# wenet-e2e/wekws

Hardware: AMD Instinct MI355X
Metric: 1-sec utterances/sec (40-d fbank -> DS-TCN posteriors), whole job; per-frame streaming latency in `latency` (higher is better)
Workload: dtype f32 in/out/accumulate; products as 3 x fp16 MFMA on block-floating hi/lo-split operands (fp32-level accuracy at any operand scale); 1 GPU; ds_tcn_h256 forward, 1024 x 1-s utterances per GPU, T=98 frames x 40-d fbank in HBM -> (B,98,2) posteriors + the streaming cache; batch_per_gpu=1024, frames=98, feat_dim=40, precision=f16x3, preheat_steps=2450, parallelism=utterance-parallel x1

## Files before the change

wekws_amd/csrc/ds256_g16.hip.h:

```cpp
#pragma once
#include <utility>

#include "ds256_w16.hip.h"

namespace wekws {

#ifdef WEKWS_G16_STAMPS
#define G16_PH_DECL long long tph[8] = {0, 0, 0, 0, 0, 0, 0, 0}; long long tlast = clock64()
#define G16_PH(id) do { long long now_ = clock64(); tph[id] += now_ - tlast; tlast = now_; } while (0)
#define G16_PH_DUMP                                                                                    \
  do {                                                                                                 \
    __syncthreads();                                                                                   \
    if (blockIdx.x == 0 && A.out_cache && (threadIdx.x & 63) == 0)                                    \
      for (int i = 0; i < 8; ++i) A.out_cache[(threadIdx.x >> 6) * 8 + i] = float(tph[i]);               \
  } while (0)
#else
#define G16_PH_DECL
#define G16_PH(id)
#define G16_PH_DUMP
#endif

template <int S>
__device__ __forceinline__ void g16_fmac_shr(float& o, float x, float w) {
  static_assert(S >= 1 && S <= 15, "row shift");
#define G16_SHR(n) if constexpr (S == n) asm("v_fmac_f32_dpp %0, %1, %2 row_shr:" #n " row_mask:0xf bank_mask:0xf" : "+v"(o) : "v"(x), "v"(w));
  G16_SHR(1) G16_SHR(2) G16_SHR(3) G16_SHR(4) G16_SHR(5) G16_SHR(6) G16_SHR(7) G16_SHR(8)
  G16_SHR(9) G16_SHR(10) G16_SHR(11) G16_SHR(12) G16_SHR(13) G16_SHR(14) G16_SHR(15)
#undef G16_SHR
}
template <int S, int TT_, int NT, int R_>
__device__ __forceinline__ void g16_tap(float& o, const f32x4 (&hv)[NT], float w) {
  constexpr int Q = S / NT, M = S % NT;
  constexpr int REG = TT_ >= M ? TT_ - M : TT_ - M + NT;
  constexpr int SH = TT_ >= M ? Q : Q + 1;
  if constexpr (SH == 0) o = fmaf(w, hv[REG][R_], o);
  else if constexpr (SH <= 15) g16_fmac_shr<SH>(o, hv[REG][R_], w);
}
template <int S, int NT, int R_, int... TTs>
__device__ __forceinline__ void g16_tap_tiles(float (&o)[NT], const f32x4 (&hv)[NT], float w, std::integer_sequence<int, TTs...>) {
  (g16_tap<S, TTs, NT, R_>(o[TTs], hv, w), ...);
}

template <int S>
__device__ __forceinline__ void g16_fmac_shl(float& o, float x, float w) {
  static_assert(S >= 1 && S <= 15, "row shift");
#define G16_SHL(n) if constexpr (S == n) asm("v_fmac_f32_dpp %0, %1, %2 row_shl:" #n " row_mask:0xf bank_mask:0xf" : "+v"(o) : "v"(x), "v"(w));
  G16_SHL(1) G16_SHL(2) G16_SHL(3) G16_SHL(4) G16_SHL(5) G16_SHL(6) G16_SHL(7) G16_SHL(8)
  G16_SHL(9) G16_SHL(10) G16_SHL(11) G16_SHL(12) G16_SHL(13) G16_SHL(14) G16_SHL(15)
#undef G16_SHL
}
template <int S, int TT_, int NT, int R_, int PART>
__device__ __forceinline__ void g16_tapc(float& o, const f32x4 (&hv)[NT], const f32x4 (&cx)[NT], float w) {
  constexpr int Q = S / NT, M = S % NT;
  constexpr int REG = TT_ >= M ? TT_ - M : TT_ - M + NT;
  constexpr int SH = TT_ >= M ? Q : Q + 1;
  static_assert(SH <= 15, "the context is one 16-lane row: NT >= 4 for paddings up to 56 frames");
  if constexpr (SH == 0) {
    if constexpr (PART == 0) o = fmaf(w, hv[REG][R_], o);
  } else if constexpr (PART == 0) {
    g16_fmac_shr<SH>(o, hv[REG][R_], w);
  } else {
    g16_fmac_shl<16 - SH>(o, cx[REG][R_], w);
  }
}
template <int S, int NT, int R_, int... TTs>
__device__ __forceinline__ void g16_tapc_tiles(float (&o)[NT], const f32x4 (&hv)[NT], const f32x4 (&cx)[NT], float w,
                                               std::integer_sequence<int, TTs...>) {
  (g16_tapc<S, TTs, NT, R_, 0>(o[TTs], hv, cx, w), ...);
  (g16_tapc<S, TTs, NT, R_, 1>(o[TTs], hv, cx, w), ...);
}

typedef float g16_f32x2 __attribute__((ext_vector_type(2)));
typedef _Float16 g16_f16x2 __attribute__((ext_vector_type(2)));

template <bool SPLIT>
__device__ __forceinline__ void g16_split_pair(float v0, float v1, float s, unsigned& ph, unsigned& pl) {
  const float t0 = fmaxf(v0, 0.f) * s, t1 = fmaxf(v1, 0.f) * s;
  const g16_f16x2 h = __builtin_convertvector(g16_f32x2{t0, t1}, g16_f16x2);
  ph = __builtin_bit_cast(unsigned, h);
  if constexpr (SPLIT) {
    const float d0 = t0 - static_cast<float>(h[0]), d1 = t1 - static_cast<float>(h[1]);
    pl = __builtin_bit_cast(unsigned, __builtin_convertvector(g16_f32x2{d0, d1}, g16_f16x2));
  }
}

template <int D, int P_, int NT, bool SPLIT, bool CTX = false>
__device__ __forceinline__ void g16_dw_pair(const f32x4 (&hv)[NT], const f32x4 (&cx)[NT], const float* taps_o0, float sa, char* pst, int lo_off) {
  const float4* src = reinterpret_cast<const float4*>(taps_o0 + 2 * P_ * 12);
  const float4 a0 = src[0], a1 = src[1], a2 = src[2], b0 = src[3], b1 = src[4], b2 = src[5];
  constexpr auto tiles = std::make_integer_sequence<int, NT>{};
  constexpr int RA = 2 * P_, RB = 2 * P_ + 1;
  float oa[NT], ob[NT];
  __builtin_amdgcn_s_setprio(P_ == 0 ? 3 : 1);
#pragma unroll
  for (int tt = 0; tt < NT; ++tt) { oa[tt] = a2.x; ob[tt] = b2.x; }
  if constexpr (CTX) {
    g16_tapc_tiles<7 * D, NT, RA>(oa, hv, cx, a0.x, tiles); g16_tapc_tiles<7 * D, NT, RB>(ob, hv, cx, b0.x, tiles);
    g16_tapc_tiles<6 * D, NT, RA>(oa, hv, cx, a0.y, tiles); g16_tapc_tiles<6 * D, NT, RB>(ob, hv, cx, b0.y, tiles);
    g16_tapc_tiles<5 * D, NT, RA>(oa, hv, cx, a0.z, tiles); g16_tapc_tiles<5 * D, NT, RB>(ob, hv, cx, b0.z, tiles);
    g16_tapc_tiles<4 * D, NT, RA>(oa, hv, cx, a0.w, tiles); g16_tapc_tiles<4 * D, NT, RB>(ob, hv, cx, b0.w, tiles);
    g16_tapc_tiles<3 * D, NT, RA>(oa, hv, cx, a1.x, tiles); g16_tapc_tiles<3 * D, NT, RB>(ob, hv, cx, b1.x, tiles);
    g16_tapc_tiles<2 * D, NT, RA>(oa, hv, cx, a1.y, tiles); g16_tapc_tiles<2 * D, NT, RB>(ob, hv, cx, b1.y, tiles);
    g16_tapc_tiles<1 * D, NT, RA>(oa, hv, cx, a1.z, tiles); g16_tapc_tiles<1 * D, NT, RB>(ob, hv, cx, b1.z, tiles);
    g16_tapc_tiles<0, NT, RA>(oa, hv, cx, a1.w, tiles);     g16_tapc_tiles<0, NT, RB>(ob, hv, cx, b1.w, tiles);
  } else {
  g16_tap_tiles<7 * D, NT, RA>(oa, hv, a0.x, tiles); g16_tap_tiles<7 * D, NT, RB>(ob, hv, b0.x, tiles);
  g16_tap_tiles<6 * D, NT, RA>(oa, hv, a0.y, tiles); g16_tap_tiles<6 * D, NT, RB>(ob, hv, b0.y, tiles);
  g16_tap_tiles<5 * D, NT, RA>(oa, hv, a0.z, tiles); g16_tap_tiles<5 * D, NT, RB>(ob, hv, b0.z, tiles);
  g16_tap_tiles<4 * D, NT, RA>(oa, hv, a0.w, tiles); g16_tap_tiles<4 * D, NT, RB>(ob, hv, b0.w, tiles);
  g16_tap_tiles<3 * D, NT, RA>(oa, hv, a1.x, tiles); g16_tap_tiles<3 * D, NT, RB>(ob, hv, b1.x, tiles);
  g16_tap_tiles<2 * D, NT, RA>(oa, hv, a1.y, tiles); g16_tap_tiles<2 * D, NT, RB>(ob, hv, b1.y, tiles);
  g16_tap_tiles<1 * D, NT, RA>(oa, hv, a1.z, tiles); g16_tap_tiles<1 * D, NT, RB>(ob, hv, b1.z, tiles);
  g16_tap_tiles<0, NT, RA>(oa, hv, a1.w, tiles);     g16_tap_tiles<0, NT, RB>(ob, hv, b1.w, tiles);
  }
  __builtin_amdgcn_s_setprio(P_ == 0 ? 2 : 0);
#pragma unroll
  for (int tt = 0; tt < NT; ++tt) {
    unsigned ph, pl;
    g16_split_pair<SPLIT>(oa[tt], ob[tt], sa, ph, pl);
    *reinterpret_cast<unsigned*>(pst + tt * 256 + P_ * 4) = ph;
    if constexpr (SPLIT) *reinterpret_cast<unsigned*>(pst + lo_off + tt * 256 + P_ * 4) = pl;
  }
}
template <int D, int NT, bool SPLIT, bool CTX = false>
__device__ __forceinline__ void g16_dw_rows(const f32x4 (&hv)[NT], const f32x4 (&cx)[NT], const float* taps_o0, float sa, char* pst, int lo_off) {
  g16_dw_pair<D, 0, NT, SPLIT, CTX>(hv, cx, taps_o0, sa, pst, lo_off);
  g16_dw_pair<D, 1, NT, SPLIT, CTX>(hv, cx, taps_o0, sa, pst, lo_off);
}
template <int D, int NT, bool SPLIT>
__device__ __forceinline__ void g16_dw_rows(const f32x4 (&hv)[NT], const float* taps_o0, float sa, char* pst, int lo_off) {
  g16_dw_rows<D, NT, SPLIT, false>(hv, hv, taps_o0, sa, pst, lo_off);
}

template <int NT>
__device__ __forceinline__ void g16_load_run(const float* src, f32x4 (&cv)[NT], int r) {
  struct __attribute__((packed, aligned(4))) V4 { float v[4]; };
  struct __attribute__((packed, aligned(4))) V3 { float v[3]; };
  if constexpr (NT == 7) {
    const V4 a = *reinterpret_cast<const V4*>(src);
    const V3 c = *reinterpret_cast<const V3*>(src + 4);
    cv[0][r] = a.v[0]; cv[1][r] = a.v[1]; cv[2][r] = a.v[2]; cv[3][r] = a.v[3];
    cv[4][r] = c.v[0]; cv[5][r] = c.v[1]; cv[6][r] = c.v[2];
  } else if constexpr (NT == 4) {
    const V4 a = *reinterpret_cast<const V4*>(src);
    cv[0][r] = a.v[0]; cv[1][r] = a.v[1]; cv[2][r] = a.v[2]; cv[3][r] = a.v[3];
  } else {
#pragma unroll
    for (int tt = 0; tt < NT; ++tt) cv[tt][r] = src[tt];
  }
}

template <int NT, int PB>
__device__ __forceinline__ W16XItem g16_take_x(const float* xbuf, int T, int idim, int nk, int e) {
  constexpr int TT = 16 * NT;
  W16XItem it;
  const int n = e % TT, q = e / TT;
  const int f = NT * (n & 15) + (n >> 4);
  const int oct = q & 3, st = q >> 2;
  const int kf = st * 32 + oct * 8;
  const bool has = e < nk * 4 * TT;
  it.dst = has ? st * 2 * PB + (oct * TT + n) * 16 : -1;
  it.ok = has && f < T && kf < idim;
  const float* p = xbuf + (it.ok ? f * idim + kf : 0);
  const float4 a = *reinterpret_cast<const float4*>(p), c = *reinterpret_cast<const float4*>(p + 4);
  it.v = w16_f32x8{a.x, a.y, a.z, a.w, c.x, c.y, c.z, c.w};
  return it;
}

template <int NT>
__device__ __forceinline__ void g16_store_run(float* dst, const f32x4 (&hv)[NT], int r) {
  struct __attribute__((packed, aligned(4))) V4 { float v[4]; };
  struct __attribute__((packed, aligned(4))) V3 { float v[3]; };
  struct __attribute__((packed, aligned(4))) V2 { float v[2]; };
  if constexpr (NT == 7) {
    *reinterpret_cast<V4*>(dst) = V4{{hv[0][r], hv[1][r], hv[2][r], hv[3][r]}};
    *reinterpret_cast<V3*>(dst + 4) = V3{{hv[4][r], hv[5][r], hv[6][r]}};
  } else if constexpr (NT == 4) {
    *reinterpret_cast<V4*>(dst) = V4{{hv[0][r], hv[1][r], hv[2][r], hv[3][r]}};
  } else if constexpr (NT == 2) {
    *reinterpret_cast<V2*>(dst) = V2{{hv[0][r], hv[1][r]}};
  } else {
#pragma unroll
    for (int tt = 0; tt < NT; ++tt) dst[tt] = hv[tt][r];
  }
}

template <int NT, int PB>
__device__ __forceinline__ W16XItem g16_load_x(const float* __restrict__ xb, int T, int idim, int nk, int e) {
  constexpr int TT = 16 * NT;
  W16XItem it;
  const int n = e % TT, q = e / TT;
  const int f = NT * (n & 15) + (n >> 4);
  const int oct = q & 3, st = q >> 2;
  const int kf = st * 32 + oct * 8;
  const bool has = e < nk * 4 * TT;
  it.dst = has ? st * 2 * PB + (oct * TT + n) * 16 : -1;
  w16_fetch_x(it, xb + int64_t(f) * idim + kf, xb, has && f < T && kf < idim);
  return it;
}

template <int NT, bool SPLIT, bool FIRST = false>
__device__ __forceinline__ void g16_mfma_step(f32x4 (&acc)[NT], const F16Frag& a, const char* bh, const char* bl) {
  f16x8 vh[2], vl[2];
  vh[0] = *reinterpret_cast<const f16x8*>(bh);
  if constexpr (SPLIT) vl[0] = *reinterpret_cast<const f16x8*>(bl);
#pragma unroll
  for (int tt = 0; tt < NT; ++tt) {
    if (tt + 1 < NT) {
      vh[(tt + 1) & 1] = *reinterpret_cast<const f16x8*>(bh + (tt + 1) * 256);
      if constexpr (SPLIT) vl[(tt + 1) & 1] = *reinterpret_cast<const f16x8*>(bl + (tt + 1) * 256);
    }
    __builtin_amdgcn_sched_barrier(0);
    acc[tt] = __builtin_amdgcn_mfma_f32_16x16x32_f16(a.h, vh[tt & 1], FIRST ? f32x4{0.f, 0.f, 0.f, 0.f} : acc[tt], 0, 0, 0);
    if constexpr (SPLIT) {
      acc[tt] = __builtin_amdgcn_mfma_f32_16x16x32_f16(a.h, vl[tt & 1], acc[tt], 0, 0, 0);
      acc[tt] = __builtin_amdgcn_mfma_f32_16x16x32_f16(a.l, vh[tt & 1], acc[tt], 0, 0, 0);
    }
    __builtin_amdgcn_sched_barrier(0);
  }
}

template <int NT, bool SPLIT, bool FAST, bool CTX = false>
__global__ __launch_bounds__(kW16Threads) void ds256_g16_kernel(const StackParams P, const CallArgs A) {
  static_assert(!CTX || (FAST && NT >= 4), "the context tile is one 16-lane row");
  using G = W16Geom<NT>;
  constexpr int C = G::C, SS = G::SS, TT = G::TT, PB = G::PB;
  constexpr int NKS = C / 32;
  constexpr int OTS = NKS * 128;
  static_assert(size_t(2 * NKS) * PB <= G::LDS_BYTES, "the operand planes of a whole layer live where the f32 tile was");
  extern __shared__ __attribute__((aligned(16))) float w16_lds[];
  char* const planes = reinterpret_cast<char*>(w16_lds);
  float* const hbuf = w16_lds + G::SLAB / 4;

  f32x4 acc[NT];
  f32x4 hv[NT];
  f32x4 cx[CTX ? NT : 1];
  G16_PH_DECL;

  __shared__ AmaxCell amax_cells[kAmaxCells];
  __shared__ BlockDesc blk[kAmaxMaxBlocks];
  __shared__ NfList nfl;
  nf_list_init(nfl);
  __shared__ __attribute__((aligned(16))) float taps[C * 12];
  const int nk = P.kpre16 / 32;
  const bool one_trip = FAST || (nk <= 2 && 8 * TT <= kW16Threads && w16_x_vec_ok(A.x, A.xs_b, P.idim));
  static_assert(kAmaxMaxBlocks * sizeof(BlockDesc) / 4 <= kW16Threads, "one table dword per thread");
  {
    const int ntbl = P.nblocks * int(sizeof(BlockDesc) / 4);
    const int t0 = threadIdx.x;
    if (t0 < ntbl) reinterpret_cast<uint32_t*>(blk)[t0] = reinterpret_cast<const uint32_t*>(P.blocks)[t0];
  }
  float* const xbuf = w16_lds + (2 * NKS * PB) / 4;
  static_assert(!FAST || size_t(2 * NKS) * PB + size_t(TT) * 64 * 4 <= G::LDS_BYTES, "feature buffer above the planes");
  auto prefetch_x = [&](int bn) __attribute__((always_inline)) {
    const int nitems = (A.T * P.idim) >> 2;
    const float* src = A.x + int64_t(bn) * A.xs_b;
    const int t0 = threadIdx.x;
    for (int e0 = 0; e0 < nitems; e0 += kW16Threads) {
      const int wbase = __builtin_amdgcn_readfirstlane(e0 + (t0 & ~63));
      if (e0 + t0 < nitems)
        __builtin_amdgcn_global_load_lds((const __attribute__((address_space(1))) void*)(src + (e0 + t0) * 4),
                                         (__attribute__((address_space(3))) void*)(xbuf + wbase * 4), 16, 0, 0);
    }
  };
  if constexpr (FAST) prefetch_x(blockIdx.x);
  for (int b = blockIdx.x; b < A.B; b += gridDim.x) {
  const float* Wp = P.w;
  if constexpr (FAST) asm volatile("" : "+s"(Wp));
  const float* __restrict__ W = Wp;
  int tid = threadIdx.x;
  if constexpr (FAST) asm volatile("" : "+v"(tid));
  const int lane = tid & 63, wave = __builtin_amdgcn_readfirstlane(tid >> 6);
  const int l15 = lane & 15, lq = lane >> 4;
  int T = A.T;
  if constexpr (FAST) asm volatile("" : "+s"(T));
  const int Pc = P.cache_len;
  const int o0 = wave * 16 + lq * 4;
  const int frag_off = (lq * TT + l15) * 16;
  char* const pst = planes + (wave >> 1) * 2 * PB + ((((wave & 1) * 2 + (lq >> 1)) * TT + l15) * 16 + (lq & 1) * 8);

  auto stage_taps = [&](const BlockDesc& nb) __attribute__((always_inline)) {
    if (wave < C * 3 / 64)
      __builtin_amdgcn_global_load_lds((const __attribute__((address_space(1))) void*)(W + nb.dw_pk + tid * 4),
                                       (__attribute__((address_space(3))) void*)(taps + wave * 256), 16, 0, 0);
  };
  auto load_ctx = [&](int bi) __attribute__((always_inline)) {
    if constexpr (CTX) {
      const int padn = __builtin_amdgcn_readfirstlane(blk[bi].pad), offn = __builtin_amdgcn_readfirstlane(blk[bi].cache_off);
      const float* const ic = A.in_cache + (int64_t(b) * C + o0) * Pc + offn;
      const int c0 = padn + NT * (l15 - 16);
#pragma unroll
      for (int tt = 0; tt < NT; ++tt) cx[tt] = f32x4{0.f, 0.f, 0.f, 0.f};
      if (c0 >= 0) {
#pragma unroll
        for (int r = 0; r < 4; ++r) g16_load_run<NT>(ic + r * Pc + c0, cx, r);
      } else if (c0 + NT > 0) {
#pragma unroll
        for (int tt = 0; tt < NT; ++tt)
          if (c0 + tt >= 0) {
#pragma unroll
            for (int r = 0; r < 4; ++r) cx[tt][r] = ic[r * Pc + c0 + tt];
          }
      }
    }
  };
  auto skip_bad = [&]() __attribute__((always_inline)) {
    nf_list_note(nfl, b);
    if constexpr (FAST) {
      if (b + int(gridDim.x) < A.B) prefetch_x(b + gridDim.x);
    }
  };
  amax_zero<kW16Threads>(amax_cells, kAmaxCells);
  W16XItem xi;
  if constexpr (!FAST) {
    if (one_trip) xi = g16_load_x<NT, PB>(A.x + int64_t(b) * A.xs_b, T, P.idim, nk, tid);
  } else {
    __builtin_amdgcn_s_waitcnt(0x0F70);
  }
  __syncthreads();
  stage_taps(blk[0]);
  if constexpr (CTX)
    amax_publish(amax_cells + 1, amax_span_bits<kW16Threads>(A.in_cache + int64_t(b) * C * Pc, C * Pc, 0.f));
  if constexpr (FAST) xi = g16_take_x<NT, PB>(xbuf, T, P.idim, nk, tid);
  if (one_trip) {
    amax_publish(amax_cells, w16_x_amax_bits(xi));
  } else {
    amax_publish(amax_cells, amax_span_bits<kW16Threads>(A.x + int64_t(b) * A.xs_b, T * P.idim, 0.f));
  }

  {
#pragma unroll
    for (int tt = 0; tt < NT; ++tt) acc[tt] = f32x4{0.f, 0.f, 0.f, 0.f};
    const uint4* ap = reinterpret_cast<const uint4*>(W + P.pre_a16) + size_t(wave) * nk * 128 + lane;
    const float4 bias = *reinterpret_cast<const float4*>(W + P.pre_b + o0);
    float sx = 1.f, cpre = 1.f;
    if (one_trip) {
      F16Frag a[2];
#pragma unroll
      for (int st = 0; st < 2; ++st) {
        const uint4* q = ap + min(st, nk - 1) * 128;
        a[st].h = __builtin_bit_cast(f16x8, q[0]);
        a[st].l = __builtin_bit_cast(f16x8, q[64]);
      }
      __syncthreads();
      if (amax_inputs_bad(amax_cells)) { skip_bad(); continue; }
      sx = pow2_scale(amax_read(amax_cells), &cpre);
      w16_store_x<PB, SPLIT>(xi, sx, planes);
      __syncthreads();
#pragma unroll
      for (int st = 0; st < 2; ++st)
        if (st < nk)
          g16_mfma_step<NT, SPLIT>(acc, a[st], planes + st * 2 * PB + frag_off, planes + st * 2 * PB + PB + frag_off);
    } else {
    __syncthreads();
    if (amax_inputs_bad(amax_cells)) { skip_bad(); continue; }
    for (int k0 = 0; k0 < nk; k0 += 2) {
      const int steps = min(2, nk - k0);
      __syncthreads();
      sx = pow2_scale(amax_read(amax_cells), &cpre);
      for (int e = tid; e < steps * 4 * TT; e += kW16Threads) {
        const int n = e % TT;
        const int t = NT * (n & 15) + (n >> 4);
        const int q = e / TT;
        const int oct = q & 3, st = q >> 2;
        const int kf = (k0 + st) * 32 + oct * 8;
        const bool ok = t < T;
        const float* xr = A.x + int64_t(b) * A.xs_b + int64_t(t) * P.idim + kf;
        f16x8 vh, vl;
#pragma unroll
        for (int i = 0; i < 8; ++i) {
          const float v = (ok && kf + i < P.idim) ? xr[i] * sx : 0.f;
          _Float16 h, l;
          split16(v, h, l);
          vh[i] = h; vl[i] = l;
        }
        char* dst = planes + st * 2 * PB + (oct * TT + n) * 16;
        *reinterpret_cast<f16x8*>(dst) = vh;
        if constexpr (SPLIT) *reinterpret_cast<f16x8*>(dst + PB) = vl;
      }
      __syncthreads();
      for (int st = 0; st < steps; ++st) {
        F16Frag a[1];
        load_a16<1>(a, ap + (k0 + st) * 128, 0);
        g16_mfma_step<NT, SPLIT>(acc, a[0], planes + st * 2 * PB + frag_off, planes + st * 2 * PB + PB + frag_off);
      }
    }
    }
    cpre *= P.pre_inv_s;
    float hmax = 0.f;
#pragma unroll
    for (int tt = 0; tt < NT; ++tt) {
#pragma unroll
      for (int r = 0; r < 4; ++r) {
        float v = fmaf(acc[tt][r], cpre, f4c(bias, r));
        if (P.pre_relu) v = fmaxf(v, 0.f);
        hv[tt][r] = v;
        hmax = fmaxf(hmax, fabsf(v));
      }
    }
    amax_publish(amax_cells + 2, hmax);
    __syncthreads();
  }
  G16_PH(0);
  F16Frag a0;
  auto frag_base = [&](int i) __attribute__((always_inline)) {
    return reinterpret_cast<const uint4*>(W + __builtin_amdgcn_readfirstlane(blk[i].a1_16)) + size_t(wave) * OTS;
  };
  {
    const uint4* ap0 = frag_base(0);
    F16Frag t[1];
    load_a16<1>(t, ap0 + lane, 0); a0 = t[0];
  }
  for (int bi = 0; bi < P.nblocks; ++bi) {
    const BlockDesc bd = blk[bi];
    const int pad = bd.pad;
    const uint4* ap1 = frag_base(bi);
    const uint4* apn = frag_base(min(bi + 1, P.nblocks - 1));
    float c1;
    const float au = CTX ? fmaxf(amax_read(amax_cells + 2 + bi), amax_read(amax_cells + 1)) : amax_read(amax_cells + 2 + bi);
    const float sa = pow2_scale(fmaf(bd.dw_alpha, au, bd.dw_beta), &c1);
    c1 *= bd.inv_s1;

    auto hand_over = [&]() __attribute__((always_inline)) {
      if (A.out_cache) {
        float* const oc = A.out_cache + (int64_t(b) * C + o0) * Pc + bd.cache_off;
        const int p0 = NT * l15 - (T - pad);
        if (p0 >= 0 && p0 + NT <= pad) {
#pragma unroll
          for (int r = 0; r < 4; ++r) g16_store_run<NT>(oc + r * Pc + p0, hv, r);
        } else if (p0 + NT > 0 && p0 < pad) {
#pragma unroll
          for (int tt = 0; tt < NT; ++tt) {
            const int p = p0 + tt;
            if (p >= 0 && p < pad) {
#pragma unroll
              for (int r = 0; r < 4; ++r) oc[r * Pc + p] = hv[tt][r];
            }
          }
        }
        if (T < pad) {
          const int nz = pad - T;
          for (int e = lane; e < 16 * nz; e += 64) {
            const int cc = e / nz, p = e - cc * nz;
            const int64_t at = (int64_t(b) * C + wave * 16 + cc) * Pc + bd.cache_off + p;
            A.out_cache[at] = CTX ? A.in_cache[at + T] : 0.f;
          }
        }
      }
    };
    load_ctx(bi);
    G16_PH(1);

    {
      const float* taps_o0 = taps + o0 * 12;
      switch (bd.dil) {
        case 1: if constexpr (CTX) g16_dw_rows<1, NT, SPLIT, true>(hv, cx, taps_o0, sa, pst, PB); else g16_dw_rows<1, NT, SPLIT>(hv, taps_o0, sa, pst, PB); break;
        case 2: if constexpr (CTX) g16_dw_rows<2, NT, SPLIT, true>(hv, cx, taps_o0, sa, pst, PB); else g16_dw_rows<2, NT, SPLIT>(hv, taps_o0, sa, pst, PB); break;
        case 4: if constexpr (CTX) g16_dw_rows<4, NT, SPLIT, true>(hv, cx, taps_o0, sa, pst, PB); else g16_dw_rows<4, NT, SPLIT>(hv, taps_o0, sa, pst, PB); break;
        case 8: if constexpr (CTX) g16_dw_rows<8, NT, SPLIT, true>(hv, cx, taps_o0, sa, pst, PB); else g16_dw_rows<8, NT, SPLIT>(hv, taps_o0, sa, pst, PB); break;
        default: break;
      }
    }
    G16_PH(2);
    __syncthreads();
    G16_PH(3);

    F16Frag a1;
    {
      F16Frag t[1];
      load_a16<1>(t, ap1 + 128 + lane, 0); a1 = t[0];
    }
    const float4 ebias = *reinterpret_cast<const float4*>(W + bd.b1 + o0);
    if (bi + 1 < P.nblocks) stage_taps(blk[bi + 1]);

    auto kpass = [&](int ks, auto first_c) __attribute__((always_inline)) {
      if (ks == 0) __builtin_amdgcn_s_setprio(3);
      else if (ks == 2) __builtin_amdgcn_s_setprio(2);
      else if (ks == 4) __builtin_amdgcn_s_setprio(1);
      else __builtin_amdgcn_s_setprio(0);
      const char* bsrc = planes + ks * 2 * PB + frag_off;
      const uint4* nx = ks + 2 < NKS ? ap1 + (ks + 2) * 128 : apn;
      g16_mfma_step<NT, SPLIT, decltype(first_c)::value>(acc, a0, bsrc, bsrc + PB);
      {
        F16Frag t[1];
        load_a16<1>(t, nx + lane, 0); a0 = t[0];
      }
      g16_mfma_step<NT, SPLIT>(acc, a1, bsrc + 2 * PB, bsrc + 3 * PB);
      if (ks + 2 < NKS) {
        F16Frag t[1];
        load_a16<1>(t, nx + 128 + lane, 0); a1 = t[0];
      }
    };
    kpass(0, std::true_type{});
#pragma unroll 1
    for (int ks = 2; ks < NKS; ks += 2) kpass(ks, std::false_type{});
    G16_PH(4);

    hand_over();
    G16_PH(6);

    float hmax = 0.f;
#pragma unroll
    for (int tt = 0; tt < NT; ++tt) {
#pragma unroll
      for (int r = 0; r < 4; ++r) {
        const float v = fmaxf(fmaf(acc[tt][r], c1, f4c(ebias, r)), 0.f) + hv[tt][r];
        hv[tt][r] = v;
        hmax = fmaxf(hmax, fabsf(v));
      }
    }
    amax_publish(amax_cells + 3 + bi, hmax);
    G16_PH(5);
    __syncthreads();
    G16_PH(3);
  }

  if (FAST || (P.head == HEAD_LINEAR && P.odim <= 2)) {
    const int K = P.odim;
    constexpr int PS = 32 * NT + 16;
    float* const part = w16_lds;
    {
      const float4 w0 = *reinterpret_cast<const float4*>(W + P.head_w + o0);
      const float4 w1 = *reinterpret_cast<const float4*>(W + P.head_w + (K > 1 ? C : 0) + o0);
      if constexpr (FAST) {
        if (b + int(gridDim.x) < A.B) prefetch_x(b + gridDim.x);
      }
      float* dst = part + (wave * 4 + lq) * PS + 2 * NT * l15;
      const HeadPairs hw(w0, w1);
#pragma unroll
      for (int tt = 0; tt < NT; ++tt) {
        pk_f32x2 pp{0.f, 0.f};
        head_fma4(pp, hw.x, hw.y, hw.z, hw.w, hv[tt]);
        *reinterpret_cast<float2*>(dst + 2 * tt) = float2{pp.x, pp.y};
      }
    }
    __syncthreads();
    {
      const int e = tid >> 2, qd = tid & 3;
      const int t = e >> 1, k = e & 1;
      const float* src = part + qd * 16 * PS + e;
      float v = 0.f;
#pragma unroll
      for (int i = 0; i < 16; ++i) v += src[i * PS];
      v += __builtin_bit_cast(float, __builtin_amdgcn_update_dpp(0, __builtin_bit_cast(int, v), 0xB1, 0xf, 0xf, true));
      v += __builtin_bit_cast(float, __builtin_amdgcn_update_dpp(0, __builtin_bit_cast(int, v), 0x4E, 0xf, 0xf, true));
      if (qd == 0 && t < T && k < K) {
        v += W[P.head_b + k];
        if (P.sigmoid) v = sigmoidf_(v);
        A.y[int64_t(b) * A.ys_b + int64_t(t) * K + k] = v;
      }
    }
  } else if constexpr (!FAST) {
#pragma unroll
    for (int tt = 0; tt < NT; ++tt) {
#pragma unroll
      for (int r = 0; r < 4; ++r) hbuf[(o0 + r) * SS + NT * l15 + tt] = hv[tt][r];
    }
    __syncthreads();
    conv_stack_head<KIND_DS, 256, NT, kW16Threads, SS>(P, A, hbuf, w16_lds, b);
  }
  G16_PH(7);
  if constexpr (!FAST) break;
  }
  nf_list_drain(nfl, A, P.idim, C * P.cache_len, blockIdx.x, gridDim.x);
  G16_PH_DUMP;
}

int launch_ds256_g16(const Route& r, const StackParams& P, const CallArgs& A, hipStream_t stream);

}
```

Measured before the change: 5.037 million utts/s.

## Use SGPR-base plus VGPR-offset global addressing and move next-utterance prefetch earlier

Weight and feature loads now go through explicit global address-space pointers, with a uniform scalar base and a 32-bit per-lane offset. This lets the compiler emit saddr+voffset global loads instead of building 64-bit per-lane addresses. The k-loop peels its final pass so the last pass never issues the unused a1 fragment load. The tap staging for the next block is moved after the MFMA loop, and the FAST-path prefetch of the next utterance is moved from the head into the last block so it overlaps more work. The risk is that the earlier prefetch writes xbuf while it may still be read, and the moved staging changes the overlap timing.

```diff
diff --git a/wekws_amd/csrc/ds256_g16.hip.h b/wekws_amd/csrc/ds256_g16.hip.h
--- a/wekws_amd/csrc/ds256_g16.hip.h
+++ b/wekws_amd/csrc/ds256_g16.hip.h
@@ -199,6 +199,33 @@
   return it;
 }
 
+#if defined(__HIP_DEVICE_COMPILE__)
+typedef const __attribute__((address_space(1))) char* g16_gptr;
+#else
+typedef const char* g16_gptr;
+#endif
+__device__ __forceinline__ g16_gptr g16_global(const void* p) { return (g16_gptr)p; }
+template <class V>
+__device__ __forceinline__ V g16_ld(g16_gptr base, uint32_t off) {
+  asm volatile("" : "+v"(off));
+#if defined(__HIP_DEVICE_COMPILE__)
+  return *reinterpret_cast<const __attribute__((address_space(1))) V*>(base + off);
+#else
+  return *reinterpret_cast<const V*>(base + off);
+#endif
+}
+__device__ __forceinline__ g16_gptr g16_sect(g16_gptr w, uint32_t at) { return w + int64_t(at) * 4; }
+__device__ __forceinline__ uint32_t g16_voff(uint32_t off) {
+  asm volatile("" : "+v"(off));
+  return off;
+}
+__device__ __forceinline__ F16Frag g16_frag(g16_gptr base, uint32_t lane_off) {
+  F16Frag a;
+  a.h = g16_ld<f16x8>(base, lane_off);
+  a.l = g16_ld<f16x8>(base + 64 * 16, lane_off);
+  return a;
+}
+
 template <int NT, bool SPLIT, bool FIRST = false>
 __device__ __forceinline__ void g16_mfma_step(f32x4 (&acc)[NT], const F16Frag& a, const char* bh, const char* bl) {
   f16x8 vh[2], vl[2];
@@ -254,20 +281,20 @@
   static_assert(!FAST || size_t(2 * NKS) * PB + size_t(TT) * 64 * 4 <= G::LDS_BYTES, "feature buffer above the planes");
   auto prefetch_x = [&](int bn) __attribute__((always_inline)) {
     const int nitems = (A.T * P.idim) >> 2;
-    const float* src = A.x + int64_t(bn) * A.xs_b;
+    const g16_gptr src = g16_global(A.x + int64_t(bn) * A.xs_b);
     const int t0 = threadIdx.x;
     for (int e0 = 0; e0 < nitems; e0 += kW16Threads) {
       const int wbase = __builtin_amdgcn_readfirstlane(e0 + (t0 & ~63));
       if (e0 + t0 < nitems)
-        __builtin_amdgcn_global_load_lds((const __attribute__((address_space(1))) void*)(src + (e0 + t0) * 4),
+        __builtin_amdgcn_global_load_lds(src + int64_t(wbase) * 16 + g16_voff(uint32_t(t0 & 63) * 16),
                                          (__attribute__((address_space(3))) void*)(xbuf + wbase * 4), 16, 0, 0);
     }
   };
   if constexpr (FAST) prefetch_x(blockIdx.x);
   for (int b = blockIdx.x; b < A.B; b += gridDim.x) {
-  const float* Wp = P.w;
-  if constexpr (FAST) asm volatile("" : "+s"(Wp));
-  const float* __restrict__ W = Wp;
+  g16_gptr Wg = g16_global(P.w);
+  if constexpr (FAST) asm volatile("" : "+s"(Wg));
+
   int tid = threadIdx.x;
   if constexpr (FAST) asm volatile("" : "+v"(tid));
   const int lane = tid & 63, wave = __builtin_amdgcn_readfirstlane(tid >> 6);
@@ -277,11 +304,12 @@
   const int Pc = P.cache_len;
   const int o0 = wave * 16 + lq * 4;
   const int frag_off = (lq * TT + l15) * 16;
+  const uint32_t lane_off = lane * 16;
   char* const pst = planes + (wave >> 1) * 2 * PB + ((((wave & 1) * 2 + (lq >> 1)) * TT + l15) * 16 + (lq & 1) * 8);
 
   auto stage_taps = [&](const BlockDesc& nb) __attribute__((always_inline)) {
     if (wave < C * 3 / 64)
-      __builtin_amdgcn_global_load_lds((const __attribute__((address_space(1))) void*)(W + nb.dw_pk + tid * 4),
+      __builtin_amdgcn_global_load_lds(g16_sect(Wg, __builtin_amdgcn_readfirstlane(nb.dw_pk)) + wave * 1024 + g16_voff(lane_off),
                                        (__attribute__((address_space(3))) void*)(taps + wave * 256), 16, 0, 0);
   };
   auto load_ctx = [&](int bi) __attribute__((always_inline)) {
@@ -331,16 +359,14 @@
   {
 #pragma unroll
     for (int tt = 0; tt < NT; ++tt) acc[tt] = f32x4{0.f, 0.f, 0.f, 0.f};
-    const uint4* ap = reinterpret_cast<const uint4*>(W + P.pre_a16) + size_t(wave) * nk * 128 + lane;
-    const float4 bias = *reinterpret_cast<const float4*>(W + P.pre_b + o0);
+    const g16_gptr ap = g16_sect(Wg, P.pre_a16) + int64_t(wave) * nk * 2048;
+    const float4 bias = g16_ld<float4>(g16_sect(Wg, P.pre_b), o0 * 4);
     float sx = 1.f, cpre = 1.f;
     if (one_trip) {
       F16Frag a[2];
 #pragma unroll
       for (int st = 0; st < 2; ++st) {
-        const uint4* q = ap + min(st, nk - 1) * 128;
-        a[st].h = __builtin_bit_cast(f16x8, q[0]);
-        a[st].l = __builtin_bit_cast(f16x8, q[64]);
+        a[st] = g16_frag(ap + min(st, nk - 1) * 2048, lane_off);
       }
       __syncthreads();
       if (amax_inputs_bad(amax_cells)) { skip_bad(); continue; }
@@ -380,9 +406,8 @@
       }
       __syncthreads();
       for (int st = 0; st < steps; ++st) {
-        F16Frag a[1];
-        load_a16<1>(a, ap + (k0 + st) * 128, 0);
-        g16_mfma_step<NT, SPLIT>(acc, a[0], planes + st * 2 * PB + frag_off, planes + st * 2 * PB + PB + frag_off);
+        const F16Frag a = g16_frag(ap + (k0 + st) * 2048, lane_off);
+        g16_mfma_step<NT, SPLIT>(acc, a, planes + st * 2 * PB + frag_off, planes + st * 2 * PB + PB + frag_off);
       }
     }
     }
@@ -404,18 +429,14 @@
   G16_PH(0);
   F16Frag a0;
   auto frag_base = [&](int i) __attribute__((always_inline)) {
-    return reinterpret_cast<const uint4*>(W + __builtin_amdgcn_readfirstlane(blk[i].a1_16)) + size_t(wave) * OTS;
+    return g16_sect(Wg, __builtin_amdgcn_readfirstlane(blk[i].a1_16)) + int64_t(wave) * OTS * 16;
   };
-  {
-    const uint4* ap0 = frag_base(0);
-    F16Frag t[1];
-    load_a16<1>(t, ap0 + lane, 0); a0 = t[0];
-  }
+  a0 = g16_frag(frag_base(0), lane_off);
   for (int bi = 0; bi < P.nblocks; ++bi) {
     const BlockDesc bd = blk[bi];
     const int pad = bd.pad;
-    const uint4* ap1 = frag_base(bi);
-    const uint4* apn = frag_base(min(bi + 1, P.nblocks - 1));
+    const g16_gptr ap1 = frag_base(bi);
+    const g16_gptr apn = frag_base(min(bi + 1, P.nblocks - 1));
     float c1;
     const float au = CTX ? fmaxf(amax_read(amax_cells + 2 + bi), amax_read(amax_cells + 1)) : amax_read(amax_cells + 2 + bi);
     const float sa = pow2_scale(fmaf(bd.dw_alpha, au, bd.dw_beta), &c1);
@@ -465,36 +486,32 @@
     __syncthreads();
     G16_PH(3);
 
-    F16Frag a1;
-    {
-      F16Frag t[1];
-      load_a16<1>(t, ap1 + 128 + lane, 0); a1 = t[0];
-    }
-    const float4 ebias = *reinterpret_cast<const float4*>(W + bd.b1 + o0);
-    if (bi + 1 < P.nblocks) stage_taps(blk[bi + 1]);
-
-    auto kpass = [&](int ks, auto first_c) __attribute__((always_inline)) {
+    F16Frag a1 = g16_frag(ap1 + 2048, lane_off);
+    const float4 ebias = g16_ld<float4>(g16_sect(Wg, __builtin_amdgcn_readfirstlane(bd.b1)), o0 * 4);
+
+    auto kpass = [&](int ks, auto first_c, auto last_c) __attribute__((always_inline)) {
       if (ks == 0) __builtin_amdgcn_s_setprio(3);
       else if (ks == 2) __builtin_amdgcn_s_setprio(2);
       else if (ks == 4) __builtin_amdgcn_s_setprio(1);
       else __builtin_amdgcn_s_setprio(0);
       const char* bsrc = planes + ks * 2 * PB + frag_off;
-      const uint4* nx = ks + 2 < NKS ? ap1 + (ks + 2) * 128 : apn;
+      const g16_gptr nx = ks + 2 < NKS ? ap1 + (ks + 2) * 2048 : apn;
       g16_mfma_step<NT, SPLIT, decltype(first_c)::value>(acc, a0, bsrc, bsrc + PB);
-      {
-        F16Frag t[1];
-        load_a16<1>(t, nx + lane, 0); a0 = t[0];
-      }
+      a0 = g16_frag(nx, lane_off);
       g16_mfma_step<NT, SPLIT>(acc, a1, bsrc + 2 * PB, bsrc + 3 * PB);
-      if (ks + 2 < NKS) {
-        F16Frag t[1];
-        load_a16<1>(t, nx + 128 + lane, 0); a1 = t[0];
-      }
+      if (!decltype(last_c)::value) a1 = g16_frag(nx + 2048, lane_off);
     };
-    kpass(0, std::true_type{});
+    kpass(0, std::true_type{}, std::false_type{});
 #pragma unroll 1
-    for (int ks = 2; ks < NKS; ks += 2) kpass(ks, std::false_type{});
+    for (int ks = 2; ks < NKS - 2; ks += 2) kpass(ks, std::false_type{}, std::false_type{});
+    kpass(NKS - 2, std::false_type{}, std::true_type{});
     G16_PH(4);
+
+    if (bi + 1 < P.nblocks) {
+      stage_taps(blk[bi + 1]);
+    } else if constexpr (FAST) {
+      if (b + int(gridDim.x) < A.B) prefetch_x(b + gridDim.x);
+    }
 
     hand_over();
     G16_PH(6);
@@ -520,11 +537,8 @@
     constexpr int PS = 32 * NT + 16;
     float* const part = w16_lds;
     {
-      const float4 w0 = *reinterpret_cast<const float4*>(W + P.head_w + o0);
-      const float4 w1 = *reinterpret_cast<const float4*>(W + P.head_w + (K > 1 ? C : 0) + o0);
-      if constexpr (FAST) {
-        if (b + int(gridDim.x) < A.B) prefetch_x(b + gridDim.x);
-      }
+      const float4 w0 = g16_ld<float4>(g16_sect(Wg, P.head_w), o0 * 4);
+      const float4 w1 = g16_ld<float4>(g16_sect(Wg, P.head_w + (K > 1 ? C : 0)), o0 * 4);
       float* dst = part + (wave * 4 + lq) * PS + 2 * NT * l15;
       const HeadPairs hw(w0, w1);
 #pragma unroll
@@ -545,7 +559,7 @@
       v += __builtin_bit_cast(float, __builtin_amdgcn_update_dpp(0, __builtin_bit_cast(int, v), 0xB1, 0xf, 0xf, true));
       v += __builtin_bit_cast(float, __builtin_amdgcn_update_dpp(0, __builtin_bit_cast(int, v), 0x4E, 0xf, 0xf, true));
       if (qd == 0 && t < T && k < K) {
-        v += W[P.head_b + k];
+        v += g16_ld<float>(g16_sect(Wg, P.head_b), k * 4);
         if (P.sigmoid) v = sigmoidf_(v);
         A.y[int64_t(b) * A.ys_b + int64_t(t) * K + k] = v;
       }
```

New measurement: 5.174 million utts/s (median of 6 runs). +2.7%, better.
